# vakurshakov/xpic

Measured on AMD Instinct MI355X. Metric: particles pushed/sec (ECSIM full step) + KSP iters/sec, 256^3 grid 64ppc, higher is better.
Workload: dtype f64

## Files before the change

### xpic_amd/csrc/fields.hip

```cpp
#include <cmath>
#include <utility>

#include "common.h"
#include "lstencil.h"

namespace xpic {

int experiment_fields() { return XPIC_TU_EXPERIMENT; }

namespace {

constexpr int kBlock = 256;

inline dim3 ew_grid(const GridDev& g)
{
  long blocks = (g.nown + kBlock * 2 - 1) / (kBlock * 2);
  if (blocks > 2048) blocks = 2048;
  if (blocks < 1) blocks = 1;
  return dim3((unsigned)blocks, 3, 1);
}

template <class F>
__global__ void __launch_bounds__(kBlock) k_ew(GridDev g, F f)
{
  const long off = (long)blockIdx.y * g.cstride + (long)g.G * g.plane;
  const long n = g.nown;
  const long stride = (long)gridDim.x * kBlock;
  for (long i = (long)blockIdx.x * kBlock + threadIdx.x; i < n; i += stride) f(off + i);
}

struct FSet { double* y; double a; __device__ void operator()(long i) const { y[i] = a; } };
struct FCopy { double* y; const double* x; __device__ void operator()(long i) const { y[i] = x[i]; } };
struct FAxpy { double* y; double a; const double* x; __device__ void operator()(long i) const { y[i] += a * x[i]; } };
struct FAxpby { double* y; double a, b; const double* x; __device__ void operator()(long i) const { y[i] = a * x[i] + b * y[i]; } };
struct FWaxpby { double* w; double a; const double* x; double b; const double* y; __device__ void operator()(long i) const { w[i] = a * x[i] + b * y[i]; } };
struct FScaleTo { double* y; double a; const double* x; __device__ void operator()(long i) const { y[i] = a * x[i]; } };

template <class F>
int launch_ew(xpic_ctx* c, F f)
{
  hipLaunchKernelGGL(k_ew<F>, ew_grid(c->g), dim3(kBlock), 0, c->stream, c->g, f);
  XPIC_HIP(hipGetLastError());
  return 0;
}

__device__ inline double wave_sum(double v)
{
  for (int o = 32; o > 0; o >>= 1) v += __shfl_down(v, o, 64);
  return v;
}

template <int NV>
__device__ inline void block_reduce_store(double (&acc)[NV], double* partial, int nblocks, int block)
{
  __shared__ double sm[NV][kBlock / 64];
  const int lane = threadIdx.x & 63, wave = threadIdx.x >> 6;
#pragma unroll
  for (int j = 0; j < NV; ++j) {
    double v = wave_sum(acc[j]);
    if (lane == 0) sm[j][wave] = v;
  }
  __syncthreads();
  if (threadIdx.x < NV) {
    double v = 0;
#pragma unroll
    for (int w = 0; w < kBlock / 64; ++w) v += sm[threadIdx.x][w];
    partial[(long)threadIdx.x * nblocks + block] = v;
  }
}

struct VPtrs { const double* p[8]; };
struct HVals { double h[8]; };

template <int NV, bool WW>
__global__ void __launch_bounds__(kBlock) k_mdot(GridDev g, const double* w, VPtrs V, double* partial)
{
  double acc[NV + (WW ? 1 : 0)];
#pragma unroll
  for (int j = 0; j < NV + (WW ? 1 : 0); ++j) acc[j] = 0.0;
  const long off = (long)blockIdx.y * g.cstride + (long)g.G * g.plane;
  const long stride = (long)gridDim.x * kBlock;
  for (long i = (long)blockIdx.x * kBlock + threadIdx.x; i < g.nown; i += stride) {
    double wi = w[off + i];
#pragma unroll
    for (int j = 0; j < NV; ++j) acc[j] += wi * V.p[j][off + i];
    if (WW) acc[NV] += wi * wi;
  }
  block_reduce_store<NV + (WW ? 1 : 0)>(acc, partial, gridDim.x * gridDim.y, blockIdx.y * gridDim.x + blockIdx.x);
}

template <int NV, bool NORM>
__global__ void __launch_bounds__(kBlock) k_maxpy(GridDev g, const double* w, VPtrs V, HVals h, double* partial, double* out,
  double scale)
{
  double acc[1] = {0.0};
  const long off = (long)blockIdx.y * g.cstride + (long)g.G * g.plane;
  const long stride = (long)gridDim.x * kBlock;
  for (long i = (long)blockIdx.x * kBlock + threadIdx.x; i < g.nown; i += stride) {
    double wi = w[off + i];
#pragma unroll
    for (int j = 0; j < NV; ++j) wi -= h.h[j] * V.p[j][off + i];
    wi *= scale;
    out[off + i] = wi;
    if (NORM) acc[0] += wi * wi;
  }
  if (NORM) block_reduce_store<1>(acc, partial, gridDim.x * gridDim.y, blockIdx.y * gridDim.x + blockIdx.x);
}

__global__ void __launch_bounds__(kBlock) k_stats(GridDev g, const double* f, double* partial)
{
  double acc[2] = {0.0, 0.0};
  const long off = (long)blockIdx.y * g.cstride + (long)g.G * g.plane;
  const long stride = (long)gridDim.x * kBlock;
  for (long i = (long)blockIdx.x * kBlock + threadIdx.x; i < g.nown; i += stride) {
    double v = f[off + i];
    acc[0] += v * v;
    acc[1] += v;
  }
  block_reduce_store<2>(acc, partial, gridDim.x * gridDim.y, blockIdx.y * gridDim.x + blockIdx.x);
}

__global__ void __launch_bounds__(kBlock) k_reduce_final(const double* partial, int nblocks, int nseg, double* out)
{
  const int j = blockIdx.x / nseg, s = blockIdx.x % nseg;
  const int seg = nblocks / nseg;
  double v = 0;
  for (int i = threadIdx.x; i < seg; i += kBlock) v += partial[(long)j * nblocks + s * seg + i];
  __shared__ double sm[kBlock / 64];
  v = wave_sum(v);
  if ((threadIdx.x & 63) == 0) sm[threadIdx.x >> 6] = v;
  __syncthreads();
  if (threadIdx.x == 0) {
    double t = 0;
    for (int w = 0; w < kBlock / 64; ++w) t += sm[w];
    out[blockIdx.x] = t;
  }
}

inline dim3 red_grid(const GridDev& g)
{
  long blocks = (g.nown + kBlock * 4 - 1) / (kBlock * 4);
  long cap = kRedBlocks / 3;
  if (blocks > cap) blocks = cap;
  if (blocks < 1) blocks = 1;
  return dim3((unsigned)blocks, 3, 1);
}

int finish_reduce(xpic_ctx* c, int nv, int nblocks, int nseg, double* host_out)
{
  hipLaunchKernelGGL(k_reduce_final, dim3(nv * nseg), dim3(kBlock), 0, c->stream, c->red_partial, nblocks, nseg, c->red_out);
  XPIC_HIP(hipGetLastError());
  XPIC_CALL(comm_allreduce_sum(c, c->red_out, nv * nseg));
  XPIC_HIP(hipMemcpyAsync(c->red_host, c->red_out, sizeof(double) * nv * nseg, hipMemcpyDeviceToHost, c->stream));
  XPIC_HIP(hipStreamSynchronize(c->stream));
  for (int i = 0; i < nv * nseg; ++i) host_out[i] = c->red_host[i];
  return 0;
}

template <int SIGN, class T = double>
__device__ inline void rot_at(const GridDev& g, const T* F, int x, int y, int z, double& rx, double& ry, double& rz)
{
  const double ix = g.inv[0], iy = g.inv[1], iz = g.inv[2];
  const T* Fx = F;
  const T* Fy = F + g.cstride;
  const T* Fz = F + 2 * g.cstride;
  const long c0 = g.nodew(x, y, z);
  if (SIGN > 0) {
    const long xp = g.nodew(x + 1, y, z), yp = g.nodew(x, y + 1, z), zp = g.nodew(x, y, z + 1);
    rx = +iy * Fz[yp] - iy * Fz[c0] - iz * Fy[zp] + iz * Fy[c0];
    ry = -ix * Fz[xp] + ix * Fz[c0] + iz * Fx[zp] - iz * Fx[c0];
    rz = +ix * Fy[xp] - ix * Fy[c0] - iy * Fx[yp] + iy * Fx[c0];
  }
  else {
    const long xm = g.nodew(x - 1, y, z), ym = g.nodew(x, y - 1, z), zm = g.nodew(x, y, z - 1);
    rx = +iy * Fz[c0] - iy * Fz[ym] - iz * Fy[c0] + iz * Fy[zm];
    ry = -ix * Fz[c0] + ix * Fz[xm] + iz * Fx[c0] - iz * Fx[zm];
    rz = +ix * Fy[c0] - ix * Fy[xm] - iy * Fx[c0] + iy * Fx[ym];
  }
}

template <int SIGN>
__global__ void __launch_bounds__(kBlock) k_rot(GridDev g, double alpha, const double* F, double* out, int add)
{
  const long n = g.nown;
  const long stride = (long)gridDim.x * kBlock;
  for (long i = (long)blockIdx.x * kBlock + threadIdx.x; i < n; i += stride) {
    int x = (int)(i % g.nx), y = (int)((i / g.nx) % g.ny), z = (int)(i / g.plane);
    double rx, ry, rz;
    rot_at<SIGN>(g, F, x, y, z, rx, ry, rz);
    const long o = g.node(x, y, g.wz(z));
    if (add) {
      out[o] += alpha * rx;
      out[o + g.cstride] += alpha * ry;
      out[o + 2 * g.cstride] += alpha * rz;
    }
    else {
      out[o] = alpha * rx;
      out[o + g.cstride] = alpha * ry;
      out[o + 2 * g.cstride] = alpha * rz;
    }
  }
}

template <class T = double>
__device__ inline void matM_at(const GridDev& g, const T* F, int x, int y, int z, double& mx, double& my, double& mz)
{
  const double ix = g.inv[0], iy = g.inv[1], iz = g.inv[2];
  double ax, ay, az;
  double bx, by, bz;
  double cx, cy, cz;
  double dx_, dy_, dz_;
  rot_at<+1, T>(g, F, x, y, z, ax, ay, az);
  rot_at<+1, T>(g, F, x - 1, y, z, bx, by, bz);
  rot_at<+1, T>(g, F, x, y - 1, z, cx, cy, cz);
  rot_at<+1, T>(g, F, x, y, z - 1, dx_, dy_, dz_);
  const double s = 0.5 * g.dt * g.dt;
  const long c0 = g.nodew(x, y, z);
  double rx = +iy * az - iy * cz - iz * ay + iz * dy_;
  double ry = -ix * az + ix * bz + iz * ax - iz * dx_;
  double rz = +ix * ay - ix * by - iy * ax + iy * cx;
  mx = 2.0 * (double)F[c0] + s * rx;
  my = 2.0 * (double)F[c0 + g.cstride] + s * ry;
  mz = 2.0 * (double)F[c0 + 2 * g.cstride] + s * rz;
}

__global__ void __launch_bounds__(kBlock) k_matM(GridDev g, const double* F, double* out, int add, int z0r, int nzr)
{
  const long n = (long)nzr * g.plane;
  const long stride = (long)gridDim.x * kBlock;
  for (long i = (long)blockIdx.x * kBlock + threadIdx.x; i < n; i += stride) {
    int x = (int)(i % g.nx), y = (int)((i / g.nx) % g.ny), z = z0r + (int)(i / g.plane);
    double mx, my, mz;
    matM_at(g, F, x, y, z, mx, my, mz);
    const long o = g.node(x, y, g.wz(z));
    if (add) { out[o] += mx; out[o + g.cstride] += my; out[o + 2 * g.cstride] += mz; }
    else { out[o] = mx; out[o + g.cstride] = my; out[o + 2 * g.cstride] = mz; }
  }
}

__global__ void __launch_bounds__(kBlock) k_cg_apply_dot(GridDev g, const double* __restrict__ p, double* __restrict__ Ap,
  double* partial)
{
  double acc[1] = {0.0};
  const long stride = (long)gridDim.x * kBlock;
  for (long i = (long)blockIdx.x * kBlock + threadIdx.x; i < g.nown; i += stride) {
    int x = (int)(i % g.nx), y = (int)((i / g.nx) % g.ny), z = (int)(i / g.plane);
    double m[3];
    matM_at(g, p, x, y, z, m[0], m[1], m[2]);
    const long o = g.node(x, y, g.wz(z));
#pragma unroll
    for (int c = 0; c < 3; ++c) {
      Ap[o + c * g.cstride] = m[c];
      acc[0] += p[o + c * g.cstride] * m[c];
    }
  }
  block_reduce_store<1>(acc, partial, gridDim.x, blockIdx.x);
}

__global__ void __launch_bounds__(kBlock) k_cg_update(GridDev g, double alpha, const double* __restrict__ p,
  const double* __restrict__ Ap, double* __restrict__ x, double* __restrict__ r, double* partial)
{
  double acc[1] = {0.0};
  const long off = (long)blockIdx.y * g.cstride + (long)g.G * g.plane;
  const long stride = (long)gridDim.x * kBlock;
  for (long i = (long)blockIdx.x * kBlock + threadIdx.x; i < g.nown; i += stride) {
    x[off + i] += alpha * p[off + i];
    const double rv = r[off + i] - alpha * Ap[off + i];
    r[off + i] = rv;
    acc[0] += rv * rv;
  }
  block_reduce_store<1>(acc, partial, gridDim.x * gridDim.y, blockIdx.y * gridDim.x + blockIdx.x);
}

template <bool FIRST>
__global__ void __launch_bounds__(kBlock) k_cheb(GridDev g, const double* __restrict__ r, const double* __restrict__ zin,
  double* __restrict__ d, double* __restrict__ zout, double cd, double cr, double itheta)
{
  const long n = g.nown;
  const long stride = (long)gridDim.x * kBlock;
  for (long i = (long)blockIdx.x * kBlock + threadIdx.x; i < n; i += stride) {
    int x = (int)(i % g.nx), y = (int)((i / g.nx) % g.ny), z = (int)(i / g.plane);
    double m[3];
    matM_at(g, FIRST ? r : zin, x, y, z, m[0], m[1], m[2]);
    const long o = g.node(x, y, g.wz(z));
#pragma unroll
    for (int c = 0; c < 3; ++c) {
      const long oc = o + c * g.cstride;
      const double rv = r[oc];
      const double z0 = FIRST ? rv * itheta : zin[oc];
      const double dn = cd * (FIRST ? z0 : d[oc]) + cr * (rv - (FIRST ? m[c] * itheta : m[c]));
      d[oc] = dn;
      zout[oc] = z0 + dn;
    }
  }
}

template <bool FIRST, bool LAST>
__global__ void __launch_bounds__(kBlock) k_cheb32(GridDev g, const double* __restrict__ r64, float* __restrict__ r32,
  const float* __restrict__ zin, float* __restrict__ d, float* __restrict__ zout, double* __restrict__ out64, double cd,
  double cr, double itheta)
{
  const long n = g.nown;
  const long stride = (long)gridDim.x * kBlock;
  for (long i = (long)blockIdx.x * kBlock + threadIdx.x; i < n; i += stride) {
    int x = (int)(i % g.nx), y = (int)((i / g.nx) % g.ny), z = (int)(i / g.plane);
    double m[3];
    if (FIRST) matM_at<double>(g, r64, x, y, z, m[0], m[1], m[2]);
    else matM_at<float>(g, zin, x, y, z, m[0], m[1], m[2]);
    const long o = g.node(x, y, g.wz(z));
#pragma unroll
    for (int c = 0; c < 3; ++c) {
      const long oc = o + c * g.cstride;
      const double rv = FIRST ? r64[oc] : (double)r32[oc];
      const double z0 = FIRST ? rv * itheta : (double)zin[oc];
      const double dn = cd * (FIRST ? z0 : (double)d[oc]) + cr * (rv - (FIRST ? m[c] * itheta : m[c]));
      if (FIRST && !LAST) r32[oc] = (float)rv;
      if (LAST) out64[oc] = z0 + dn;
      else {
        d[oc] = (float)dn;
        zout[oc] = (float)(z0 + dn);
      }
    }
  }
}


constexpr int kRowX = 64, kRowY = 4;
constexpr int kBandY = 4;

template <int C1>
struct XTile {
  static constexpr int nx(int c2) { return lrange(C1, c2).n[0] + kRowX - 1; }
  static constexpr int ny(int c2) { return lrange(C1, c2).n[1] + kRowY - 1; }
  static constexpr int nz(int c2) { return lrange(C1, c2).n[2]; }
  static constexpr int off(int c2)
  {
    int o = 0;
    for (int c = 0; c < c2; ++c) o += nx(c) * ny(c) * nz(c);
    return o;
  }
  static constexpr int size = off(3);
  static constexpr int at(int c2, int dx, int dy, int dz)
  {
    const LRange r = lrange(C1, c2);
    return off(c2) + ((dz - r.lo[2]) * ny(c2) + (dy - r.lo[1])) * nx(c2) + (dx - r.lo[0]);
  }
};
constexpr int kXTileMax = XTile<0>::size > XTile<1>::size ? (XTile<0>::size > XTile<2>::size ? XTile<0>::size : XTile<2>::size)
                                                          : (XTile<1>::size > XTile<2>::size ? XTile<1>::size : XTile<2>::size);
static_assert(kXTileMax * 8 <= 40960 - 1280, "four workgroups of k_matA per CU: 160 KB of LDS");

__device__ __forceinline__ int fold_or_zero(int v, int n)
{
  v = v < 0 ? v + n : (v >= n ? v - n : v);
  return v < n ? v : 0;
}

template <int C1, int C2>
__device__ __forceinline__ void xtile_fill_c(const GridDev& g, const double* __restrict__ X, double* tile, int x0, int y0, int z, int tx, int w)
{
  constexpr LRange r = lrange(C1, C2);
  constexpr int NX = XTile<C1>::nx(C2), NY = XTile<C1>::ny(C2), NZ = XTile<C1>::nz(C2), OFF = XTile<C1>::off(C2);
  static_assert(NX > kRowX && NX <= 2 * kRowX, "a tile row is one full and one partial pass of the wave");
  const int gx0 = fold_or_zero(x0 + r.lo[0] + tx, g.nx), gx1 = fold_or_zero(x0 + r.lo[0] + kRowX + tx, g.nx);
  for (int row = w; row < NY * NZ; row += kRowY) {
    const int pz = row / NY, py = row - pz * NY;
    const double* src = X + C2 * g.cstride + (long)g.wz(z + r.lo[2] + pz) * g.plane + (long)fold_or_zero(y0 + r.lo[1] + py, g.ny) * g.nx;
    tile[OFF + row * NX + tx] = src[gx0];
    if (tx < NX - kRowX) tile[OFF + row * NX + kRowX + tx] = src[gx1];
  }
}

#ifndef MATA_GROUP
#define MATA_GROUP 12
#endif
#ifndef MATA_DEPTH
#define MATA_DEPTH 2
#endif
constexpr int kLGroup = MATA_GROUP, kLDepth = MATA_DEPTH;

struct RowAddr {
  unsigned xl8[kLDepth];
  int lb[3];
};

template <int C1, int K>
__device__ __forceinline__ void lterm(double (&acc)[2], const char* Lb, RowAddr& a, const double* tile)
{
  constexpr LEntry e = ldecode(C1, K);
  constexpr int toff = XTile<C1>::at(e.c2, e.d[0], e.d[1], e.d[2]);
  constexpr int set = (K / kLGroup) % kLDepth;
  const double xv = tile[a.lb[e.c2] + toff];
  const double lv = *reinterpret_cast<const double*>(Lb + (size_t)K * 32 + a.xl8[set]);
  acc[K & 1] += lv * xv;
  if (K % kLGroup == kLGroup - 1)
    asm volatile("" : "+v"(a.xl8[set]), "+v"(a.lb[0]), "+v"(a.lb[1]), "+v"(a.lb[2]) : "v"(acc[0]), "v"(acc[1]));
}

template <int C1, int... Ks>
__device__ __forceinline__ double row_apply(std::integer_sequence<int, Ks...>, const GridDev& g, const double* __restrict__ L,
  const double* tile, const int (&lb)[3], int x, int y, int z)
{
  const char* Lb = reinterpret_cast<const char*>(L + g.lindex(C1, z + (g.G ? 1 : 0), y, 0, 0));
  RowAddr a;
  for (int d = 0; d < kLDepth; ++d) a.xl8[d] = (unsigned)(x >> 2) * (8u * kLBlock) + 8u * (unsigned)(x & 3);
  for (int c = 0; c < 3; ++c) a.lb[c] = lb[c];
  double acc[2] = {0.0, 0.0};
  (lterm<C1, Ks>(acc, Lb, a, tile), ...);
  return acc[0] + acc[1];
}

template <int C, class At>
__device__ __forceinline__ double matM_comp(const GridDev& g, At at)
{
  constexpr int A = (C + 1) % 3, B = (C + 2) % 3;
  const double ih[3] = {g.inv[0], g.inv[1], g.inv[2]};
  auto sh = [&](int axis, int s, int& ox, int& oy, int& oz) { (axis == 0 ? ox : (axis == 1 ? oy : oz)) += s; };
  auto dplus = [&](int comp, int axis, int ox, int oy, int oz) {
    int px = ox, py = oy, pz = oz;
    sh(axis, +1, px, py, pz);
    return (at(comp, px, py, pz) - at(comp, ox, oy, oz)) * ih[axis];
  };
  auto GB = [&](int ox, int oy, int oz) { return dplus(A, C, ox, oy, oz) - dplus(C, A, ox, oy, oz); };
  auto GA = [&](int ox, int oy, int oz) { return dplus(C, B, ox, oy, oz) - dplus(B, C, ox, oy, oz); };
  int ax = 0, ay = 0, az = 0, bx = 0, by = 0, bz = 0;
  sh(A, -1, ax, ay, az);
  sh(B, -1, bx, by, bz);
  const double r = (GB(0, 0, 0) - GB(ax, ay, az)) * ih[A] - (GA(0, 0, 0) - GA(bx, by, bz)) * ih[B];
  return 2.0 * at(C, 0, 0, 0) + (0.5 * g.dt * g.dt) * r;
}

template <bool WITH_M, int C1>
__device__ __forceinline__ void rows_of(const GridDev& g, const double* __restrict__ L, const double* __restrict__ X,
  double* __restrict__ Y, double* tile, int add, int x0, int y0, int z, int tx, int ty)
{
  xtile_fill_c<C1, 0>(g, X, tile, x0, y0, z, tx, ty);
  xtile_fill_c<C1, 1>(g, X, tile, x0, y0, z, tx, ty);
  xtile_fill_c<C1, 2>(g, X, tile, x0, y0, z, tx, ty);
  __syncthreads();
  const int x = x0 + tx, y = y0 + ty;
  if (x >= g.nx || y >= g.ny) return;
  const int lb[3] = {ty * XTile<C1>::nx(0) + tx, ty * XTile<C1>::nx(1) + tx, ty * XTile<C1>::nx(2) + tx};
  double r = 0.0;
  if (WITH_M) r = matM_comp<C1>(g, [&](int comp, int ox, int oy, int oz) { return tile[lb[comp] + XTile<C1>::at(comp, ox, oy, oz)]; });
  r += row_apply<C1>(std::make_integer_sequence<int, kLStencil>{}, g, L, tile, lb, x, y, z);
  const long o = C1 * g.cstride + g.node(x, y, g.wz(z));
  if (add) Y[o] += r;
  else Y[o] = r;
}

template <bool WITH_M>
__global__ void __launch_bounds__(kRowX* kRowY, 4) k_matA(GridDev g, const double* __restrict__ L,
  const double* __restrict__ X, double* __restrict__ Y, int add, int z0r, int nzr, int zsplit)
{
  __shared__ double tile[kXTileMax];
  const int nxc = (g.nx + kRowX - 1) / kRowX, nyc = (g.ny + kRowY - 1) / kRowY;
  const int nyt = (nyc + kBandY - 1) / kBandY;
  const int ysplit = 8 / zsplit;
  const int Pz = (nzr + zsplit - 1) / zsplit;
  const int Pb = (nyt + ysplit - 1) / ysplit;
  const int per_z = kBandY * nxc * 3, per_band = Pz * per_z;
  const int xcd = blockIdx.x % 8;
  const long q = blockIdx.x / 8;
  const int ytl = (int)(q / per_band);
  const int yt = (xcd / zsplit) * Pb + ytl;
  const int rem = (int)(q % per_band);
  const int zr = (xcd % zsplit) * Pz + rem / per_z;
  const int z = z0r + zr;
  const int rem2 = rem % per_z;
  const int c1 = rem2 % 3;
  const int x0 = ((rem2 / 3) % nxc) * kRowX;
  const int y0 = (yt * kBandY + rem2 / (3 * nxc)) * kRowY;
  if (ytl >= Pb || yt >= nyt || zr >= nzr) return;
  const int tx = threadIdx.x, ty = __builtin_amdgcn_readfirstlane(threadIdx.y);
  if (c1 == 0) rows_of<WITH_M, 0>(g, L, X, Y, tile, add, x0, y0, z, tx, ty);
  else if (c1 == 1) rows_of<WITH_M, 1>(g, L, X, Y, tile, add, x0, y0, z, tx, ty);
  else rows_of<WITH_M, 2>(g, L, X, Y, tile, add, x0, y0, z, tx, ty);
}

__global__ void __launch_bounds__(kBlock) k_div_neg_add(GridDev g, const double* __restrict__ v, double* out)
{
  const double ix = g.inv[0], iy = g.inv[1], iz = g.inv[2];
  const long stride = (long)gridDim.x * kBlock;
  for (long i = (long)blockIdx.x * kBlock + threadIdx.x; i < g.nown; i += stride) {
    int x = (int)(i % g.nx), y = (int)((i / g.nx) % g.ny), z = (int)(i / g.plane);
    const long c0 = g.nodew(x, y, z);
    const double dv = +ix * v[c0] - ix * v[g.nodew(x - 1, y, z)] + iy * v[g.cstride + c0] -
      iy * v[g.cstride + g.nodew(x, y - 1, z)] + iz * v[2 * g.cstride + c0] - iz * v[2 * g.cstride + g.nodew(x, y, z - 1)];
    out[c0] += dv;
  }
}

__global__ void __launch_bounds__(kBlock) k_norm12(GridDev g, const double* f, double* partial)
{
  double acc[2] = {0.0, 0.0};
  const long off = (long)g.G * g.plane;
  const long stride = (long)gridDim.x * kBlock;
  for (long i = (long)blockIdx.x * kBlock + threadIdx.x; i < g.nown; i += stride) {
    const double v = f[off + i];
    acc[0] += fabs(v);
    acc[1] += v * v;
  }
  block_reduce_store<2>(acc, partial, gridDim.x, blockIdx.x);
}

__global__ void __launch_bounds__(kBlock) k_import(GridDev g, const double* aos, double* soa)
{
  const long n = g.nown * 3;
  const long stride = (long)gridDim.x * kBlock;
  for (long i = (long)blockIdx.x * kBlock + threadIdx.x; i < n; i += stride) {
    long node = i / 3;
    int c = (int)(i % 3);
    soa[c * g.cstride + (long)g.G * g.plane + node] = aos[i];
  }
}

__global__ void __launch_bounds__(kBlock) k_export(GridDev g, const double* soa, double* aos)
{
  const long n = g.nown * 3;
  const long stride = (long)gridDim.x * kBlock;
  for (long i = (long)blockIdx.x * kBlock + threadIdx.x; i < n; i += stride) {
    long node = i / 3;
    int c = (int)(i % 3);
    aos[i] = soa[c * g.cstride + (long)g.G * g.plane + node];
  }
}

}

int vec_set(xpic_ctx* c, double* y, double a) { return launch_ew(c, FSet{y, a}); }
int vec_copy(xpic_ctx* c, double* y, const double* x) { return launch_ew(c, FCopy{y, x}); }
int vec_axpy(xpic_ctx* c, double* y, double a, const double* x) { return launch_ew(c, FAxpy{y, a, x}); }
int vec_axpby(xpic_ctx* c, double* y, double a, double b, const double* x) { return launch_ew(c, FAxpby{y, a, b, x}); }
int vec_waxpby(xpic_ctx* c, double* w, double a, const double* x, double b, const double* y) { return launch_ew(c, FWaxpby{w, a, x, b, y}); }
int vec_scale_to(xpic_ctx* c, double* y, double a, const double* x) { return launch_ew(c, FScaleTo{y, a, x}); }

int vec_mdot_ww_host(xpic_ctx* c, const double* w, const double* V, int nv, double* out, double* ww)
{
  Timed t(c, "mdot");
  dim3 grid = red_grid(c->g);
  const int nblocks = grid.x * grid.y;
  for (int j0 = 0; j0 < nv; j0 += 8) {
    int m = nv - j0 < 8 ? nv - j0 : 8;
    const bool last = j0 + 8 >= nv && ww;
    VPtrs P{};
    for (int j = 0; j < m; ++j) P.p[j] = V + (long)(j0 + j) * c->nvec;
    double* part = c->red_partial + (long)j0 * nblocks;
    switch (m) {
#define CASE(N)                                                                                           \
  case N:                                                                                                 \
    if (last) hipLaunchKernelGGL((k_mdot<N, true>), grid, dim3(kBlock), 0, c->stream, c->g, w, P, part);  \
    else hipLaunchKernelGGL((k_mdot<N, false>), grid, dim3(kBlock), 0, c->stream, c->g, w, P, part);      \
    break;
      CASE(1) CASE(2) CASE(3) CASE(4) CASE(5) CASE(6) CASE(7) CASE(8)
#undef CASE
    }
    XPIC_HIP(hipGetLastError());
  }
  if (!ww) return finish_reduce(c, nv, nblocks, 1, out);
  double tmp[kMaxDots + 1];
  XPIC_CALL(finish_reduce(c, nv + 1, nblocks, 1, tmp));
  for (int i = 0; i < nv; ++i) out[i] = tmp[i];
  *ww = tmp[nv];
  return 0;
}

int vec_mdot_host(xpic_ctx* c, const double* w, const double* V, int nv, double* out)
{
  return vec_mdot_ww_host(c, w, V, nv, out, nullptr);
}

int vec_dot_host(xpic_ctx* c, const double* x, const double* y, double* out)
{
  return vec_mdot_host(c, x, y, 1, out);
}

int vec_maxpy_scaled(xpic_ctx* c, const double* w, const double* V, int nv, const double* h, double* out, double scale,
  double* nrm2)
{
  Timed t(c, "maxpy");
  dim3 grid = red_grid(c->g);
  const int nblocks = grid.x * grid.y;
  const double* src = w;
  for (int j0 = 0; j0 < nv; j0 += 8) {
    int m = nv - j0 < 8 ? nv - j0 : 8;
    const bool lastg = j0 + 8 >= nv;
    const bool last = lastg && nrm2;
    VPtrs P{};
    HVals H{};
    for (int j = 0; j < m; ++j) { P.p[j] = V + (long)(j0 + j) * c->nvec; H.h[j] = h[j0 + j]; }
    const double sc = lastg ? scale : 1.0;
    switch (m) {
#define CASE(N)                                                                                                \
  case N:                                                                                                      \
    if (last) hipLaunchKernelGGL((k_maxpy<N, true>), grid, dim3(kBlock), 0, c->stream, c->g, src, P, H, c->red_partial, out, sc); \
    else hipLaunchKernelGGL((k_maxpy<N, false>), grid, dim3(kBlock), 0, c->stream, c->g, src, P, H, c->red_partial, out, sc);     \
    break;
      CASE(1) CASE(2) CASE(3) CASE(4) CASE(5) CASE(6) CASE(7) CASE(8)
#undef CASE
    }
    XPIC_HIP(hipGetLastError());
    src = out;
  }
  if (nrm2) return finish_reduce(c, 1, nblocks, 1, nrm2);
  return 0;
}

int vec_maxpy_norm_host(xpic_ctx* c, double* w, const double* V, int nv, const double* h, double* nrm2)
{
  return vec_maxpy_scaled(c, w, V, nv, h, w, 1.0, nrm2);
}

int vec_maxpy(xpic_ctx* c, double* x, const double* V, int nv, const double* y)
{
  double neg[kMaxDots];
  for (int i = 0; i < nv; ++i) neg[i] = -y[i];
  return vec_maxpy_norm_host(c, x, V, nv, neg, nullptr);
}

int field_stats_host(xpic_ctx* c, const double* f, double* sumsq, double* mean3)
{
  dim3 grid = red_grid(c->g);
  const int nblocks = grid.x * grid.y;
  hipLaunchKernelGGL(k_stats, grid, dim3(kBlock), 0, c->stream, c->g, f, c->red_partial);
  XPIC_HIP(hipGetLastError());
  double out[6];
  XPIC_CALL(finish_reduce(c, 2, nblocks, 3, out));
  *sumsq = out[0] + out[1] + out[2];
  mean3[0] = out[3]; mean3[1] = out[4]; mean3[2] = out[5];
  return 0;
}

int cg_apply_dot_host(xpic_ctx* c, const double* p, double* Ap, double* pAp)
{
  Timed t(c, "matM_apply");
  long blocks = (c->g.nown + kBlock - 1) / kBlock;
  if (blocks > kRedBlocks) blocks = kRedBlocks;
  hipLaunchKernelGGL(k_cg_apply_dot, dim3((unsigned)blocks), dim3(kBlock), 0, c->stream, c->g, p, Ap, c->red_partial);
  XPIC_HIP(hipGetLastError());
  return finish_reduce(c, 1, (int)blocks, 1, pAp);
}

int cg_update_host(xpic_ctx* c, double alpha, const double* p, const double* Ap, double* x, double* r, double* rr)
{
  dim3 grid = red_grid(c->g);
  hipLaunchKernelGGL(k_cg_update, grid, dim3(kBlock), 0, c->stream, c->g, alpha, p, Ap, x, r, c->red_partial);
  XPIC_HIP(hipGetLastError());
  return finish_reduce(c, 1, grid.x * grid.y, 1, rr);
}

int rot_apply(xpic_ctx* c, int sign, double alpha, const double* x, double* y, bool add)
{
  Timed t(c, "rot_apply");
  long blocks = (c->g.nown + kBlock - 1) / kBlock;
  if (blocks > 65536) blocks = 65536;
  if (sign > 0) hipLaunchKernelGGL(k_rot<+1>, dim3((unsigned)blocks), dim3(kBlock), 0, c->stream, c->g, alpha, x, y, add ? 1 : 0);
  else hipLaunchKernelGGL(k_rot<-1>, dim3((unsigned)blocks), dim3(kBlock), 0, c->stream, c->g, alpha, x, y, add ? 1 : 0);
  XPIC_HIP(hipGetLastError());
  return 0;
}

static int matM_planes(xpic_ctx* c, const double* x, double* y, bool add, int z0r, int nzr)
{
  if (nzr <= 0) return 0;
  long blocks = ((long)nzr * c->g.plane + kBlock - 1) / kBlock;
  if (blocks > 65536) blocks = 65536;
  hipLaunchKernelGGL(k_matM, dim3((unsigned)blocks), dim3(kBlock), 0, c->stream, c->g, x, y, add ? 1 : 0, z0r, nzr);
  XPIC_HIP(hipGetLastError());
  return 0;
}

int matM_apply(xpic_ctx* c, const double* x, double* y, bool add)
{
  Timed t(c, "matM_apply");
  return matM_planes(c, x, y, add, 0, c->g.nzl);
}

static int row_split(const GridDev& g, int nzr)
{
  const long nyc = (g.ny + kRowY - 1) / kRowY, nyt = (nyc + kBandY - 1) / kBandY;
  int best = 8;
  long cost = -1;
  for (int zs = 8; zs >= 1; zs >>= 1) {
    const long load = ((nzr + zs - 1) / zs) * ((nyt + 8 / zs - 1) / (8 / zs));
    if (cost < 0 || load < cost) { cost = load; best = zs; }
  }
  return best;
}

static dim3 row_grid(const GridDev& g, int nzr, int zsplit)
{
  const long nxc = (g.nx + kRowX - 1) / kRowX, nyc = (g.ny + kRowY - 1) / kRowY;
  const long nyt = (nyc + kBandY - 1) / kBandY;
  const long Pz = (nzr + zsplit - 1) / zsplit, Pb = (nyt + 8 / zsplit - 1) / (8 / zsplit);
  return dim3((unsigned)(8 * Pb * Pz * kBandY * nxc * 3));
}

int matL_apply(xpic_ctx* c, const double* x, double* y, bool add)
{
  Timed t(c, "matL_apply");
  const int zs = row_split(c->g, c->g.nzl);
  hipLaunchKernelGGL((k_matA<false>), row_grid(c->g, c->g.nzl, zs), dim3(kRowX, kRowY), 0, c->stream, c->g, c->matL, x, y,
    add ? 1 : 0, 0, c->g.nzl, zs);
  XPIC_HIP(hipGetLastError());
  return 0;
}

static int matA_planes(xpic_ctx* c, const double* x, double* y, int z0r, int nzr)
{
  if (nzr <= 0) return 0;
  const int zs = row_split(c->g, nzr);
  hipLaunchKernelGGL((k_matA<true>), row_grid(c->g, nzr, zs), dim3(kRowX, kRowY), 0, c->stream, c->g, c->matL, x, y, 0, z0r,
    nzr, zs);
  XPIC_HIP(hipGetLastError());
  return 0;
}

int matA_apply(xpic_ctx* c, const double* x, double* y)
{
  Timed t(c, "matA_apply");
  return matA_planes(c, x, y, 0, c->g.nzl);
}

int halo_post(xpic_ctx* c, double* f, int width);
int halo_wait(xpic_ctx* c);

int op_apply_overlapped(xpic_ctx* c, bool with_L, double* x, double* y)
{
  const GridDev& g = c->g;
  const int w = with_L ? 2 : 1;
  Timed t(c, with_L ? "matA_apply" : "matM_apply");
  const int nin = g.nzl - 2 * w;
  XPIC_CALL(halo_post(c, x, w));
  if (with_L) XPIC_CALL(matA_planes(c, x, y, w, nin));
  else XPIC_CALL(matM_planes(c, x, y, false, w, nin));
  XPIC_CALL(halo_wait(c));
  const int nb = nin >= 0 ? w : g.nzl / 2;
  const int ztop = nin >= 0 ? g.nzl - w : nb;
  if (with_L) { XPIC_CALL(matA_planes(c, x, y, 0, nb)); XPIC_CALL(matA_planes(c, x, y, ztop, g.nzl - ztop)); }
  else { XPIC_CALL(matM_planes(c, x, y, false, 0, nb)); XPIC_CALL(matM_planes(c, x, y, false, ztop, g.nzl - ztop)); }
  return 0;
}

int halo_fill_f32(xpic_ctx* c, float* f, int width);

int cheb_matM_inverse(xpic_ctx* c, const double* r, double* out, int degree)
{
  Timed t(c, "precond");
  const GridDev& g = c->g;
  const double a = 2.0, b = 2.0 + 2.0 * g.dt * g.dt * (1.0 / (g.dx * g.dx) + 1.0 / (g.dy * g.dy) + 1.0 / (g.dz * g.dz));
  const double theta = 0.5 * (b + a), delta = 0.5 * (b - a), sigma1 = theta / delta;
  if (degree <= 1) return launch_ew(c, FScaleTo{out, 1.0 / theta, r});
  if (c->profiling) c->prof["cheb_steps"].launches += degree - 1;
  double rho = 1.0 / sigma1;
  long blocks = (g.nown + kBlock - 1) / kBlock;
  if (blocks > 65536) blocks = 65536;
  const dim3 grid((unsigned)blocks), block(kBlock);
  if (c->precond != 2) {
    float* d = (float*)c->kry_p[0];
    float* z0 = (float*)c->kry_p[1];
    float* z1 = (float*)c->kry_p[2];
    float* r32 = (float*)c->kry_t;
    for (int i = 1; i < degree; ++i) {
      const double rho_new = 1.0 / (2.0 * sigma1 - rho);
      const double cd = rho_new * rho, cr = 2.0 * rho_new / delta, it = 1.0 / theta;
      const bool first = i == 1, last = i == degree - 1;
      if (first) XPIC_CALL(halo_fill(c, const_cast<double*>(r), 1));
      else XPIC_CALL(halo_fill_f32(c, z0, 1));
      if (first && last) hipLaunchKernelGGL((k_cheb32<true, true>), grid, block, 0, c->stream, g, r, r32, z0, d, z1, out, cd, cr, it);
      else if (first) hipLaunchKernelGGL((k_cheb32<true, false>), grid, block, 0, c->stream, g, r, r32, z0, d, z1, out, cd, cr, it);
      else if (last) hipLaunchKernelGGL((k_cheb32<false, true>), grid, block, 0, c->stream, g, r, r32, z0, d, z1, out, cd, cr, it);
      else hipLaunchKernelGGL((k_cheb32<false, false>), grid, block, 0, c->stream, g, r, r32, z0, d, z1, out, cd, cr, it);
      XPIC_HIP(hipGetLastError());
      rho = rho_new;
      std::swap(z0, z1);
    }
    return 0;
  }
  double* d = c->kry_p[0];
  double* z0 = c->kry_p[1];
  double* z1 = c->kry_p[2];
  for (int i = 1; i < degree; ++i) {
    const double rho_new = 1.0 / (2.0 * sigma1 - rho);
    double* zout = i == degree - 1 ? out : z1;
    if (i == 1) {
      XPIC_CALL(halo_fill(c, const_cast<double*>(r), 1));
      hipLaunchKernelGGL(k_cheb<true>, grid, block, 0, c->stream, g, r, r, d, zout,
        rho_new * rho, 2.0 * rho_new / delta, 1.0 / theta);
    }
    else {
      XPIC_CALL(halo_fill(c, z0, 1));
      hipLaunchKernelGGL(k_cheb<false>, grid, block, 0, c->stream, g, r, z0, d, zout,
        rho_new * rho, 2.0 * rho_new / delta, 1.0 / theta);
    }
    XPIC_HIP(hipGetLastError());
    rho = rho_new;
    std::swap(z0, z1);
  }
  return 0;
}

int div_neg_add(xpic_ctx* c, double* v3, double* out_scalar)
{
  XPIC_CALL(halo_fill(c, v3, 1));
  long blocks = (c->g.nown + kBlock - 1) / kBlock;
  if (blocks > 65536) blocks = 65536;
  hipLaunchKernelGGL(k_div_neg_add, dim3((unsigned)blocks), dim3(kBlock), 0, c->stream, c->g, v3, out_scalar);
  XPIC_HIP(hipGetLastError());
  return 0;
}

int scalar_norm12_host(xpic_ctx* c, const double* f, double* out2)
{
  long blocks = (c->g.nown + kBlock * 4 - 1) / (kBlock * 4);
  if (blocks > kRedBlocks) blocks = kRedBlocks;
  if (blocks < 1) blocks = 1;
  hipLaunchKernelGGL(k_norm12, dim3((unsigned)blocks), dim3(kBlock), 0, c->stream, c->g, f, c->red_partial);
  XPIC_HIP(hipGetLastError());
  XPIC_CALL(finish_reduce(c, 2, (int)blocks, 1, out2));
  out2[1] = std::sqrt(out2[1]);
  return 0;
}

int field_import(xpic_ctx* c, double* dst, const double* src_host)
{
  const long n = c->g.nown * 3;
  double* tmp = nullptr;
  XPIC_HIP(hipMalloc(&tmp, sizeof(double) * n));
  XPIC_HIP(hipMemcpyAsync(tmp, src_host, sizeof(double) * n, hipMemcpyHostToDevice, c->stream));
  long blocks = (n + kBlock - 1) / kBlock;
  if (blocks > 65536) blocks = 65536;
  hipLaunchKernelGGL(k_import, dim3((unsigned)blocks), dim3(kBlock), 0, c->stream, c->g, tmp, dst);
  XPIC_HIP(hipGetLastError());
  XPIC_HIP(hipStreamSynchronize(c->stream));
  XPIC_HIP(hipFree(tmp));
  return 0;
}

int field_export(xpic_ctx* c, const double* src, double* dst_host)
{
  const long n = c->g.nown * 3;
  double* tmp = nullptr;
  XPIC_HIP(hipMalloc(&tmp, sizeof(double) * n));
  long blocks = (n + kBlock - 1) / kBlock;
  if (blocks > 65536) blocks = 65536;
  hipLaunchKernelGGL(k_export, dim3((unsigned)blocks), dim3(kBlock), 0, c->stream, c->g, src, tmp);
  XPIC_HIP(hipGetLastError());
  XPIC_HIP(hipMemcpyAsync(dst_host, tmp, sizeof(double) * n, hipMemcpyDeviceToHost, c->stream));
  XPIC_HIP(hipStreamSynchronize(c->stream));
  XPIC_HIP(hipFree(tmp));
  return 0;
}

namespace {

template <int OP, class T = double>
__global__ void __launch_bounds__(kBlock) k_planes(GridDev g, T* f, T* buf0, int zs00, T* buf1, int zs01, int width)
{
  T* buf = blockIdx.y == 0 ? buf0 : buf1;
  const int zs0 = blockIdx.y == 0 ? zs00 : zs01;
  const long per = (long)width * g.plane;
  const long n = 3 * per;
  const long stride = (long)gridDim.x * kBlock;
  for (long i = (long)blockIdx.x * kBlock + threadIdx.x; i < n; i += stride) {
    const int c = (int)(i / per);
    const long o = c * g.cstride + (long)zs0 * g.plane + (i % per);
    if (OP == 0) buf[i] = f[o];
    else if (OP == 1) f[o] = buf[i];
    else f[o] += buf[i];
  }
}

__global__ void __launch_bounds__(kBlock) k_add_into(double* dst, const double* src, long n)
{
  const long stride = (long)gridDim.x * kBlock;
  for (long i = (long)blockIdx.x * kBlock + threadIdx.x; i < n; i += stride) dst[i] += src[i];
}

inline unsigned plane_grid(long n)
{
  long b = (n + kBlock - 1) / kBlock;
  if (b > 4096) b = 4096;
  if (b < 1) b = 1;
  return (unsigned)b;
}

}

int ensure_halo_buf(xpic_ctx* c, size_t bytes)
{
  if (c->halo_bytes >= bytes) return 0;
  for (int i = 0; i < 4; ++i) {
    if (c->halo_buf[i]) XPIC_HIP(hipFree(c->halo_buf[i]));
    XPIC_HIP(hipMalloc(&c->halo_buf[i], bytes));
  }
  c->halo_bytes = bytes;
  return 0;
}

namespace {
template <class T>
int halo_fill_t(xpic_ctx* c, T* f, int width)
{
  const GridDev& g = c->g;
  if (g.G == 0) return 0;
  XPIC_CHECK(width <= g.G && width <= g.nzl, "halo width exceeds the ghost layer");
  Timed t(c, "halo");
  const long n = 3L * width * g.plane;
  const size_t bytes = sizeof(T) * n;
  XPIC_CALL(ensure_halo_buf(c, bytes));
  const unsigned nb = plane_grid(n);
  T* hb[4] = {(T*)c->halo_buf[0], (T*)c->halo_buf[1], (T*)c->halo_buf[2], (T*)c->halo_buf[3]};
  hipLaunchKernelGGL((k_planes<0, T>), dim3(nb, 2), dim3(kBlock), 0, c->stream, g, f, hb[0], g.G, hb[1], g.G + g.nzl - width, width);
  XPIC_HIP(hipGetLastError());
  XPIC_CALL(comm_ring(c, c->halo_buf[0], bytes, c->halo_buf[1], bytes, c->halo_buf[2], bytes, c->halo_buf[3], bytes));
  hipLaunchKernelGGL((k_planes<1, T>), dim3(nb, 2), dim3(kBlock), 0, c->stream, g, f, hb[2], g.G + g.nzl, hb[3], g.G - width, width);
  XPIC_HIP(hipGetLastError());
  return 0;
}
}

int halo_fill(xpic_ctx* c, double* f, int width) { return halo_fill_t<double>(c, f, width); }

int halo_fill2(xpic_ctx* c, double* f0, double* f1, int width)
{
  const GridDev& g = c->g;
  if (g.G == 0) return 0;
  XPIC_CHECK(width <= g.G && width <= g.nzl, "halo width exceeds the ghost layer");
  Timed t(c, "halo");
  const long n = 3L * width * g.plane;
  const size_t bytes = sizeof(double) * n;
  XPIC_CALL(ensure_halo_buf(c, 2 * bytes));
  const unsigned nb = plane_grid(n);
  double* hb[4] = {c->halo_buf[0], c->halo_buf[1], c->halo_buf[2], c->halo_buf[3]};
  double* fs[2] = {f0, f1};
  for (int k = 0; k < 2; ++k)
    hipLaunchKernelGGL((k_planes<0, double>), dim3(nb, 2), dim3(kBlock), 0, c->stream, g, fs[k], hb[0] + k * n, g.G, hb[1] + k * n, g.G + g.nzl - width, width);
  XPIC_HIP(hipGetLastError());
  XPIC_CALL(comm_ring(c, hb[0], 2 * bytes, hb[1], 2 * bytes, hb[2], 2 * bytes, hb[3], 2 * bytes));
  for (int k = 0; k < 2; ++k)
    hipLaunchKernelGGL((k_planes<1, double>), dim3(nb, 2), dim3(kBlock), 0, c->stream, g, fs[k], hb[2] + k * n, g.G + g.nzl, hb[3] + k * n, g.G - width, width);
  XPIC_HIP(hipGetLastError());
  return 0;
}

int halo_post(xpic_ctx* c, double* f, int width)
{
  const GridDev& g = c->g;
  if (g.G == 0) return 0;
  if (c->comm.kind != 1 || !c->comm_stream) return halo_fill(c, f, width);
  XPIC_CHECK(width <= g.G && width <= g.nzl, "halo width exceeds the ghost layer");
  const long n = 3L * width * g.plane;
  const size_t bytes = sizeof(double) * n;
  XPIC_CALL(ensure_halo_buf(c, bytes));
  const unsigned nb = plane_grid(n);
  double* hb[4] = {c->halo_buf[0], c->halo_buf[1], c->halo_buf[2], c->halo_buf[3]};
  hipLaunchKernelGGL((k_planes<0, double>), dim3(nb, 2), dim3(kBlock), 0, c->stream, g, f, hb[0], g.G, hb[1], g.G + g.nzl - width, width);
  XPIC_HIP(hipGetLastError());
  XPIC_HIP(hipEventRecord(c->comm_ev[0], c->stream));
  XPIC_HIP(hipStreamWaitEvent(c->comm_stream, c->comm_ev[0], 0));
  hipStream_t compute = c->stream;
  c->stream = c->comm_stream;
  int rc = comm_ring(c, hb[0], bytes, hb[1], bytes, hb[2], bytes, hb[3], bytes);
  if (rc == 0) {
    hipLaunchKernelGGL((k_planes<1, double>), dim3(nb, 2), dim3(kBlock), 0, c->stream, g, f, hb[2], g.G + g.nzl, hb[3], g.G - width, width);
  }
  c->stream = compute;
  XPIC_CALL(rc);
  XPIC_HIP(hipGetLastError());
  XPIC_HIP(hipEventRecord(c->comm_ev[1], c->comm_stream));
  c->halo_posted = true;
  return 0;
}

int halo_wait(xpic_ctx* c)
{
  if (!c->halo_posted) return 0;
  c->halo_posted = false;
  XPIC_HIP(hipStreamWaitEvent(c->stream, c->comm_ev[1], 0));
  return 0;
}
int halo_fill_f32(xpic_ctx* c, float* f, int width) { return halo_fill_t<float>(c, f, width); }

int halo_add(xpic_ctx* c, double* f, int width)
{
  const GridDev& g = c->g;
  if (g.G == 0) return 0;
  XPIC_CHECK(width <= g.G && width <= g.nzl, "halo width exceeds the ghost layer");
  XPIC_CHECK(2 * width <= g.nzl, "halo_add: the slab is thinner than its two halo layers");
  Timed t(c, "halo");
  const long n = 3L * width * g.plane;
  const size_t bytes = sizeof(double) * n;
  XPIC_CALL(ensure_halo_buf(c, bytes));
  const unsigned nb = plane_grid(n);
  hipLaunchKernelGGL(k_planes<0>, dim3(nb, 2), dim3(kBlock), 0, c->stream, g, f, c->halo_buf[0], g.G - width, c->halo_buf[1], g.G + g.nzl, width);
  XPIC_HIP(hipGetLastError());
  XPIC_CALL(comm_ring(c, c->halo_buf[0], bytes, c->halo_buf[1], bytes, c->halo_buf[2], bytes, c->halo_buf[3], bytes));
  hipLaunchKernelGGL(k_planes<2>, dim3(nb, 2), dim3(kBlock), 0, c->stream, g, f, c->halo_buf[2], g.G + g.nzl - width, c->halo_buf[3], g.G, width);
  XPIC_HIP(hipGetLastError());
  return 0;
}

int matL_ghost_rows_post(xpic_ctx* c)
{
  const GridDev& g = c->g;
  if (g.G == 0) return 0;
  XPIC_CHECK(c->lrow_buf[0] && c->lrow_buf[1], "matL ghost-row buffers missing");
  XPIC_CHECK(!c->lrow_posted, "matL ghost rows posted twice");
  Timed t(c, "matL_ghost_rows");
  const long per = g.lplane();
  const size_t bytes = sizeof(double) * per;
  const int nzp = g.nzl + 2;
  if (c->peer_copy && c->peer_lrow[0] && c->peer_lrow[1] && c->copy_stream) {
    XPIC_HIP(hipEventRecord(c->copy_ev[0], c->stream));
    XPIC_HIP(hipStreamWaitEvent(c->copy_stream, c->copy_ev[0], 0));
    for (int c1 = 0; c1 < 3; ++c1) {
      double* base = c->matL + (long)c1 * nzp * per;
      if (c1 == 2) XPIC_HIP(hipMemcpyAsync(c->peer_lrow[0] + (long)c1 * per, base, bytes, hipMemcpyDefault, c->copy_stream));
      XPIC_HIP(hipMemcpyAsync(c->peer_lrow[1] + (long)c1 * per, base + (long)(nzp - 1) * per, bytes, hipMemcpyDefault, c->copy_stream));
    }
    XPIC_HIP(hipEventRecord(c->copy_ev[1], c->copy_stream));
    c->comm.sent_msgs += 4; c->comm.sent_bytes += (int64_t)(4 * bytes);
    if (c->profiling) c->prof["peer_copies"].launches += 4;
    c->peer_pending = true;
    c->peer_exchanges = 0;
    c->lrow_posted = true; c->lrow_by_copy = true; c->lrow_on_comm_stream = false;
    return 0;
  }
  c->lrow_by_copy = false;
  const bool side = c->overlap_lrows && c->comm.kind == 1 && c->comm_stream;
  hipStream_t compute = c->stream;
  if (side) {
    XPIC_HIP(hipEventRecord(c->comm_ev[0], c->stream));
    XPIC_HIP(hipStreamWaitEvent(c->comm_stream, c->comm_ev[0], 0));
    c->stream = c->comm_stream;
  }
  int rc = 0;
  for (int c1 = 0; c1 < 3 && rc == 0; ++c1) {
    double* base = c->matL + (long)c1 * nzp * per;
    const size_t down = c1 == 2 ? bytes : 0;
    rc = comm_ring(c, base, down, base + (long)(nzp - 1) * per, bytes, c->lrow_buf[0] + (long)c1 * per, down,
      c->lrow_buf[1] + (long)c1 * per, bytes);
  }
  c->stream = compute;
  XPIC_CALL(rc);
  if (side) XPIC_HIP(hipEventRecord(c->comm_ev[1], c->comm_stream));
  c->lrow_posted = true;
  c->lrow_on_comm_stream = side;
  return 0;
}

int matL_ghost_rows_finish(xpic_ctx* c)
{
  const GridDev& g = c->g;
  if (g.G == 0) return 0;
  if (!c->lrow_posted) XPIC_CALL(matL_ghost_rows_post(c));
  Timed t(c, "matL_ghost_rows");
  if (c->lrow_on_comm_stream) XPIC_HIP(hipStreamWaitEvent(c->stream, c->comm_ev[1], 0));
  if (c->lrow_by_copy && c->peer_exchanges == 0) {
    double* w = c->red_out + 124;
    XPIC_CALL(comm_ring(c, w, sizeof(double), w + 1, sizeof(double), w + 2, sizeof(double), w + 3, sizeof(double)));
  }
  c->lrow_by_copy = false;
  c->lrow_posted = false;
  const long per = g.lplane();
  const int nzp = g.nzl + 2;
  for (int c1 = 0; c1 < 3; ++c1) {
    double* base = c->matL + (long)c1 * nzp * per;
    if (c1 == 2) hipLaunchKernelGGL(k_add_into, dim3(plane_grid(per)), dim3(kBlock), 0, c->stream, base + (long)g.nzl * per, c->lrow_buf[0] + (long)c1 * per, per);
    hipLaunchKernelGGL(k_add_into, dim3(plane_grid(per)), dim3(kBlock), 0, c->stream, base + per, c->lrow_buf[1] + (long)c1 * per, per);
  }
  XPIC_HIP(hipGetLastError());
  return 0;
}

int matL_exchange_ghost_rows(xpic_ctx* c)
{
  XPIC_CALL(matL_ghost_rows_post(c));
  return matL_ghost_rows_finish(c);
}

}
```

Baseline: 6.071 billion.

## Share one union X tile across all three output components in k_matA

Previously each workgroup handled one output component c1 and loaded its own per-(c1,c2) halo tile of X, so the three components of the same x/y/z tile reloaded overlapping X data three times. Now one workgroup of 12 waves loads a single union tile covering the stencil ranges for all c1, and each group of four waves computes one component from it. This cuts global reads of X and the grid size by three. In exchange the LDS tile and the workgroup are larger, occupancy bounds change from 4 to 6 waves per SIMD, and some halo entries are loaded that a given component does not use.

After: 6.096 billion, median of 5. Within noise of the previous version (+0.4%).

```diff
diff --git a/xpic_amd/csrc/fields.hip b/xpic_amd/csrc/fields.hip
--- a/xpic_amd/csrc/fields.hip
+++ b/xpic_amd/csrc/fields.hip
@@ -328,27 +328,29 @@
 constexpr int kRowX = 64, kRowY = 4;
 constexpr int kBandY = 4;
 
-template <int C1>
-struct XTile {
-  static constexpr int nx(int c2) { return lrange(C1, c2).n[0] + kRowX - 1; }
-  static constexpr int ny(int c2) { return lrange(C1, c2).n[1] + kRowY - 1; }
-  static constexpr int nz(int c2) { return lrange(C1, c2).n[2]; }
-  static constexpr int off(int c2)
-  {
-    int o = 0;
-    for (int c = 0; c < c2; ++c) o += nx(c) * ny(c) * nz(c);
-    return o;
-  }
-  static constexpr int size = off(3);
+constexpr int kRowC = 3 * kRowY;
+struct UTile {
+  static constexpr int lo(int c2, int axis) { return axis == c2 ? -2 : -1; }
+  static constexpr int nx = 4 + kRowX - 1, ny = 4 + kRowY - 1, nz = 4;
+  static constexpr int rows = ny * nz;
+  static constexpr int size = 3 * rows * nx;
   static constexpr int at(int c2, int dx, int dy, int dz)
   {
-    const LRange r = lrange(C1, c2);
-    return off(c2) + ((dz - r.lo[2]) * ny(c2) + (dy - r.lo[1])) * nx(c2) + (dx - r.lo[0]);
+    return ((c2 * nz + dz - lo(c2, 2)) * ny + (dy - lo(c2, 1))) * nx + (dx - lo(c2, 0));
   }
 };
-constexpr int kXTileMax = XTile<0>::size > XTile<1>::size ? (XTile<0>::size > XTile<2>::size ? XTile<0>::size : XTile<2>::size)
-                                                          : (XTile<1>::size > XTile<2>::size ? XTile<1>::size : XTile<2>::size);
-static_assert(kXTileMax * 8 <= 40960 - 1280, "four workgroups of k_matA per CU: 160 KB of LDS");
+constexpr bool utile_covers()
+{
+  for (int c1 = 0; c1 < 3; ++c1)
+    for (int c2 = 0; c2 < 3; ++c2)
+      for (int a = 0; a < 3; ++a) {
+        const LRange r = lrange(c1, c2);
+        if (r.lo[a] < UTile::lo(c2, a) || r.lo[a] + r.n[a] > UTile::lo(c2, a) + 4) return false;
+      }
+  return true;
+}
+static_assert(utile_covers(), "the union of lrange(c1, c2) over c1: 4 nodes per axis from -1, from -2 along c2");
+static_assert(UTile::size * 8 <= 81920 - 1280, "two workgroups of 12 waves of k_matA per CU: 160 KB of LDS");
 
 __device__ __forceinline__ int fold_or_zero(int v, int n)
 {
@@ -356,18 +358,21 @@
   return v < n ? v : 0;
 }
 
-template <int C1, int C2>
-__device__ __forceinline__ void xtile_fill_c(const GridDev& g, const double* __restrict__ X, double* tile, int x0, int y0, int z, int tx, int w)
-{
-  constexpr LRange r = lrange(C1, C2);
-  constexpr int NX = XTile<C1>::nx(C2), NY = XTile<C1>::ny(C2), NZ = XTile<C1>::nz(C2), OFF = XTile<C1>::off(C2);
-  static_assert(NX > kRowX && NX <= 2 * kRowX, "a tile row is one full and one partial pass of the wave");
-  const int gx0 = fold_or_zero(x0 + r.lo[0] + tx, g.nx), gx1 = fold_or_zero(x0 + r.lo[0] + kRowX + tx, g.nx);
-  for (int row = w; row < NY * NZ; row += kRowY) {
-    const int pz = row / NY, py = row - pz * NY;
-    const double* src = X + C2 * g.cstride + (long)g.wz(z + r.lo[2] + pz) * g.plane + (long)fold_or_zero(y0 + r.lo[1] + py, g.ny) * g.nx;
-    tile[OFF + row * NX + tx] = src[gx0];
-    if (tx < NX - kRowX) tile[OFF + row * NX + kRowX + tx] = src[gx1];
+__device__ __forceinline__ void utile_fill(const GridDev& g, const double* __restrict__ X, double* tile, int x0, int y0, int z, int tx, int w)
+{
+  static_assert(UTile::nx > kRowX && UTile::nx <= 2 * kRowX, "a tile row is one full and one partial pass of the wave");
+  static_assert(3 * UTile::rows % kRowC == 0, "every wave fills as many tile rows");
+  const int ga0 = fold_or_zero(x0 - 1 + tx, g.nx), ga1 = fold_or_zero(x0 - 1 + kRowX + tx, g.nx);
+  const int gb0 = fold_or_zero(x0 - 2 + tx, g.nx), gb1 = fold_or_zero(x0 - 2 + kRowX + tx, g.nx);
+#pragma unroll
+  for (int i = 0; i < 3 * UTile::rows / kRowC; ++i) {
+    const int row = w + i * kRowC;
+    const int c2 = row / UTile::rows, rz = row - c2 * UTile::rows;
+    const int pz = rz / UTile::ny, py = rz - pz * UTile::ny;
+    const double* src = X + c2 * g.cstride + (long)g.wz(z + (c2 == 2 ? -2 : -1) + pz) * g.plane +
+      (long)fold_or_zero(y0 + (c2 == 1 ? -2 : -1) + py, g.ny) * g.nx;
+    tile[row * UTile::nx + tx] = src[c2 == 0 ? gb0 : ga0];
+    if (tx < UTile::nx - kRowX) tile[row * UTile::nx + kRowX + tx] = src[c2 == 0 ? gb1 : ga1];
   }
 }
 
@@ -381,30 +386,30 @@
 
 struct RowAddr {
   unsigned xl8[kLDepth];
-  int lb[3];
+  int lb;
 };
 
 template <int C1, int K>
 __device__ __forceinline__ void lterm(double (&acc)[2], const char* Lb, RowAddr& a, const double* tile)
 {
   constexpr LEntry e = ldecode(C1, K);
-  constexpr int toff = XTile<C1>::at(e.c2, e.d[0], e.d[1], e.d[2]);
+  constexpr int toff = UTile::at(e.c2, e.d[0], e.d[1], e.d[2]);
   constexpr int set = (K / kLGroup) % kLDepth;
-  const double xv = tile[a.lb[e.c2] + toff];
+  const double xv = tile[a.lb + toff];
   const double lv = *reinterpret_cast<const double*>(Lb + (size_t)K * 32 + a.xl8[set]);
   acc[K & 1] += lv * xv;
   if (K % kLGroup == kLGroup - 1)
-    asm volatile("" : "+v"(a.xl8[set]), "+v"(a.lb[0]), "+v"(a.lb[1]), "+v"(a.lb[2]) : "v"(acc[0]), "v"(acc[1]));
+    asm volatile("" : "+v"(a.xl8[set]), "+v"(a.lb) : "v"(acc[0]), "v"(acc[1]));
 }
 
 template <int C1, int... Ks>
 __device__ __forceinline__ double row_apply(std::integer_sequence<int, Ks...>, const GridDev& g, const double* __restrict__ L,
-  const double* tile, const int (&lb)[3], int x, int y, int z)
+  const double* tile, int lb, int x, int y, int z)
 {
   const char* Lb = reinterpret_cast<const char*>(L + g.lindex(C1, z + (g.G ? 1 : 0), y, 0, 0));
   RowAddr a;
   for (int d = 0; d < kLDepth; ++d) a.xl8[d] = (unsigned)(x >> 2) * (8u * kLBlock) + 8u * (unsigned)(x & 3);
-  for (int c = 0; c < 3; ++c) a.lb[c] = lb[c];
+  a.lb = lb;
   double acc[2] = {0.0, 0.0};
   (lterm<C1, Ks>(acc, Lb, a, tile), ...);
   return acc[0] + acc[1];
@@ -431,18 +436,11 @@
 }
 
 template <bool WITH_M, int C1>
-__device__ __forceinline__ void rows_of(const GridDev& g, const double* __restrict__ L, const double* __restrict__ X,
-  double* __restrict__ Y, double* tile, int add, int x0, int y0, int z, int tx, int ty)
-{
-  xtile_fill_c<C1, 0>(g, X, tile, x0, y0, z, tx, ty);
-  xtile_fill_c<C1, 1>(g, X, tile, x0, y0, z, tx, ty);
-  xtile_fill_c<C1, 2>(g, X, tile, x0, y0, z, tx, ty);
-  __syncthreads();
-  const int x = x0 + tx, y = y0 + ty;
-  if (x >= g.nx || y >= g.ny) return;
-  const int lb[3] = {ty * XTile<C1>::nx(0) + tx, ty * XTile<C1>::nx(1) + tx, ty * XTile<C1>::nx(2) + tx};
+__device__ __forceinline__ void row_of(const GridDev& g, const double* __restrict__ L, double* __restrict__ Y,
+  const double* tile, int add, int x, int y, int z, int lb)
+{
   double r = 0.0;
-  if (WITH_M) r = matM_comp<C1>(g, [&](int comp, int ox, int oy, int oz) { return tile[lb[comp] + XTile<C1>::at(comp, ox, oy, oz)]; });
+  if (WITH_M) r = matM_comp<C1>(g, [&](int comp, int ox, int oy, int oz) { return tile[lb + UTile::at(comp, ox, oy, oz)]; });
   r += row_apply<C1>(std::make_integer_sequence<int, kLStencil>{}, g, L, tile, lb, x, y, z);
   const long o = C1 * g.cstride + g.node(x, y, g.wz(z));
   if (add) Y[o] += r;
@@ -450,16 +448,16 @@
 }
 
 template <bool WITH_M>
-__global__ void __launch_bounds__(kRowX* kRowY, 4) k_matA(GridDev g, const double* __restrict__ L,
+__global__ void __launch_bounds__(kRowX* kRowC, 6) k_matA(GridDev g, const double* __restrict__ L,
   const double* __restrict__ X, double* __restrict__ Y, int add, int z0r, int nzr, int zsplit)
 {
-  __shared__ double tile[kXTileMax];
+  __shared__ double tile[UTile::size];
   const int nxc = (g.nx + kRowX - 1) / kRowX, nyc = (g.ny + kRowY - 1) / kRowY;
   const int nyt = (nyc + kBandY - 1) / kBandY;
   const int ysplit = 8 / zsplit;
   const int Pz = (nzr + zsplit - 1) / zsplit;
   const int Pb = (nyt + ysplit - 1) / ysplit;
-  const int per_z = kBandY * nxc * 3, per_band = Pz * per_z;
+  const int per_z = kBandY * nxc, per_band = Pz * per_z;
   const int xcd = blockIdx.x % 8;
   const long q = blockIdx.x / 8;
   const int ytl = (int)(q / per_band);
@@ -468,14 +466,19 @@
   const int zr = (xcd % zsplit) * Pz + rem / per_z;
   const int z = z0r + zr;
   const int rem2 = rem % per_z;
-  const int c1 = rem2 % 3;
-  const int x0 = ((rem2 / 3) % nxc) * kRowX;
-  const int y0 = (yt * kBandY + rem2 / (3 * nxc)) * kRowY;
+  const int x0 = (rem2 % nxc) * kRowX;
+  const int y0 = (yt * kBandY + rem2 / nxc) * kRowY;
   if (ytl >= Pb || yt >= nyt || zr >= nzr) return;
-  const int tx = threadIdx.x, ty = __builtin_amdgcn_readfirstlane(threadIdx.y);
-  if (c1 == 0) rows_of<WITH_M, 0>(g, L, X, Y, tile, add, x0, y0, z, tx, ty);
-  else if (c1 == 1) rows_of<WITH_M, 1>(g, L, X, Y, tile, add, x0, y0, z, tx, ty);
-  else rows_of<WITH_M, 2>(g, L, X, Y, tile, add, x0, y0, z, tx, ty);
+  const int tx = threadIdx.x, w = __builtin_amdgcn_readfirstlane(threadIdx.y);
+  utile_fill(g, X, tile, x0, y0, z, tx, w);
+  __syncthreads();
+  const int c1 = w / kRowY, ty = w - c1 * kRowY;
+  const int x = x0 + tx, y = y0 + ty;
+  if (x >= g.nx || y >= g.ny) return;
+  const int lb = ty * UTile::nx + tx;
+  if (c1 == 0) row_of<WITH_M, 0>(g, L, Y, tile, add, x, y, z, lb);
+  else if (c1 == 1) row_of<WITH_M, 1>(g, L, Y, tile, add, x, y, z, lb);
+  else row_of<WITH_M, 2>(g, L, Y, tile, add, x, y, z, lb);
 }
 
 __global__ void __launch_bounds__(kBlock) k_div_neg_add(GridDev g, const double* __restrict__ v, double* out)
@@ -693,14 +696,14 @@
   const long nxc = (g.nx + kRowX - 1) / kRowX, nyc = (g.ny + kRowY - 1) / kRowY;
   const long nyt = (nyc + kBandY - 1) / kBandY;
   const long Pz = (nzr + zsplit - 1) / zsplit, Pb = (nyt + 8 / zsplit - 1) / (8 / zsplit);
-  return dim3((unsigned)(8 * Pb * Pz * kBandY * nxc * 3));
+  return dim3((unsigned)(8 * Pb * Pz * kBandY * nxc));
 }
 
 int matL_apply(xpic_ctx* c, const double* x, double* y, bool add)
 {
   Timed t(c, "matL_apply");
   const int zs = row_split(c->g, c->g.nzl);
-  hipLaunchKernelGGL((k_matA<false>), row_grid(c->g, c->g.nzl, zs), dim3(kRowX, kRowY), 0, c->stream, c->g, c->matL, x, y,
+  hipLaunchKernelGGL((k_matA<false>), row_grid(c->g, c->g.nzl, zs), dim3(kRowX, kRowC), 0, c->stream, c->g, c->matL, x, y,
     add ? 1 : 0, 0, c->g.nzl, zs);
   XPIC_HIP(hipGetLastError());
   return 0;
@@ -710,7 +713,7 @@
 {
   if (nzr <= 0) return 0;
   const int zs = row_split(c->g, nzr);
-  hipLaunchKernelGGL((k_matA<true>), row_grid(c->g, nzr, zs), dim3(kRowX, kRowY), 0, c->stream, c->g, c->matL, x, y, 0, z0r,
+  hipLaunchKernelGGL((k_matA<true>), row_grid(c->g, nzr, zs), dim3(kRowX, kRowC), 0, c->stream, c->g, c->matL, x, y, 0, z0r,
     nzr, zs);
   XPIC_HIP(hipGetLastError());
   return 0;
```
